# huang-yh/GaussianFormer

Measured on AMD Instinct MI355X. Metric: Gaussians/sec splatted into 200×200×16×18 voxel grid (fwd), higher is better.
Workload: dtype f32

## Files before the change

gaussianformer_amd/csrc/splat_fwd.hip:

```cpp
#include <algorithm>
#include <atomic>
#include <chrono>

#include "gf_common.hpp"

#ifndef GF_TIMELINE
#define GF_TIMELINE 0
#endif
#ifndef GF_X
#define GF_X 0
#endif
#ifndef GF_VD1
#define GF_VD1 1
#endif
#ifndef GF_PHITAB
#define GF_PHITAB 1
#endif
#ifndef GF_STATIC2
#define GF_STATIC2 0
#endif
#ifndef GF_XP
#define GF_XP 0
#endif

// ... 1485 lines not shown
                            for (int k = 0; k < 2; ++k) acc[b0 + k] = __builtin_amdgcn_mfma_f32_32x32x16_f16(sh[kh].v, wh[k][kh].v, acc[b0 + k], 0, 0, 0);
                        }
                    };
                    pair(0);
                    pair(2);
#if GF_TIMELINE
                    asm volatile("" :: "v"(acc[0]), "v"(acc[1]), "v"(acc[2]), "v"(acc[3]));
                    const unsigned long long tg3 = __builtin_amdgcn_s_memtime();
                    tacc[0] += tg1 - tg0; tacc[1] += tg2 - tg1; tacc[2] += tg3 - tg2; tacc[3] += 1;
#endif
                    qhead = (qhead + qn) & (kQCap - 1);
                    qlen -= qn;
                    npend = nnext;
                }
            }
            if (done) {
                if (last_zg && wave == 0) {
                    if (!claim_issued && lane == 0)
                        asm volatile("global_atomic_add %0, %1, %2, off sc0" : "=v"(claimed) : "v"(ctr), "v"(1u) : "memory");
                    asm volatile("s_waitcnt vmcnt(0)" : "+v"(claimed) :: "memory");
                    if (lane == 0) s_next = (int)claimed;
                }
                break;
            }
            __syncthreads();
            __builtin_amdgcn_s_setprio(3);
            list_len = 0;
        }
#if GF_TIMELINE
        if (a.timeline && tid == 0) a.timeline[4 * (size_t)logical + 2] = wall_clock64();
#endif
        if (!LABELS || a.out_logits) {
            typedef __attribute__((address_space(1))) float gfloat;
            typedef float nt4v __attribute__((ext_vector_type(4), aligned(4)));
            typedef __attribute__((address_space(1))) nt4v nt4;
            if ((a.D & 3) == 0) {
                float *stage = &s_stage[wave][0][0];
#pragma unroll
                for (int b = 0; b < 4; ++b) {
                    float *row = stage + ((b >> 1) * 64 + 32 * (b & 1) + n) * kC;
                    *reinterpret_cast<float2 *>(row + 4 * h) = make_float2(acc[b][0], acc[b][1]);
                    *reinterpret_cast<float2 *>(row + 4 * h + 2) = make_float2(acc[b][2], acc[b][3]);
                    *reinterpret_cast<float2 *>(row + 8 + 4 * h) = make_float2(acc[b][4], acc[b][5]);
                    *reinterpret_cast<float2 *>(row + 10 + 4 * h) = make_float2(acc[b][6], acc[b][7]);
                    if (h == 0) *reinterpret_cast<float2 *>(row + 16) = make_float2(acc[b][8], acc[b][9]);
                }
                uint32_t off[10];
                uint32_t okbits = 0u;
#pragma unroll
                for (int it = 0; it < 10; ++it) {
                    const int half = it / 5, i = lane + 64 * (it % 5);
                    const int run = i / kC, k = i - run * kC;
                    const int cx = Xw + (run >> 2), cy = Y0 + (run & 3), Zb = Zw + 4 * half;
                    const bool ok = i < 16 * kC && cx < a.H && cy < a.W && Zb < a.D;
                    okbits |= ok ? (1u << it) : 0u;
                    off[it] = ok ? (uint32_t)((((size_t)cx * a.W + cy) * a.D + Zb) * kC + 4 * k) : 0u;
                }
                asm volatile("" : "+v"(off[0]), "+v"(off[1]), "+v"(off[2]), "+v"(off[3]), "+v"(off[4]), "+v"(off[5]), "+v"(off[6]),
                             "+v"(off[7]), "+v"(off[8]), "+v"(off[9]));
                __builtin_amdgcn_fence(__ATOMIC_ACQ_REL, "wavefront");
                __builtin_amdgcn_wave_barrier();
                gfloat *base = (gfloat *)a.out_logits;
#pragma unroll
                for (int it = 0; it < 10; ++it) {
                    if (okbits & (1u << it)) {
                        const float4 v = *reinterpret_cast<const float4 *>(stage + (it / 5) * 64 * kC + 4 * (lane + 64 * (it % 5)));
                        __builtin_nontemporal_store((nt4v){v.x, v.y, v.z, v.w}, (nt4 *)(base + off[it]));
                    }
                }
            } else {
                float *stage = &s_stage[wave][0][0];
#pragma unroll
                for (int b = 0; b < 4; ++b) {
                    float *row = stage + ((b >> 1) * 64 + 32 * (b & 1) + n) * kC;
#pragma unroll
                    for (int r = 0; r < 10; ++r) {
                        const int c = (r & 3) + 8 * (r >> 2) + 4 * h;
                        if (c < kC) row[c] = acc[b][r];
                    }
                }
                __builtin_amdgcn_fence(__ATOMIC_ACQ_REL, "wavefront");
                __builtin_amdgcn_wave_barrier();
                for (int i = lane; i < 2 * 64 * kC; i += 64) {
                    const int half = i / (64 * kC), l = (i % (64 * kC)) / kC, ch = i % kC;
                    const int cx = Xw + (l >> 4), cy = Y0 + ((l >> 2) & 3), cz = Zw + 4 * half + (l & 3);
                    if (cx < a.H && cy < a.W && cz < a.D) a.out_logits[(((size_t)cx * a.W + cy) * a.D + cz) * kC + ch] = stage[i];
                }
            }
        }
        if (!last_zg) {
            __syncthreads();
        }
#if GF_TIMELINE
        if (a.timeline && tid == 0) a.timeline[4 * (size_t)logical + 3] = wall_clock64();
#endif
    }
#if GF_TIMELINE
    if (a.timeline && lane == 0) {
        unsigned long long *dst = a.timeline + 5 * (size_t)nslots + ((size_t)logical * 4 + wave) * 6;
        dst[0] = tacc[0]; dst[1] = tacc[1]; dst[2] = tacc[2]; dst[3] = tacc[3]; dst[4] = __builtin_amdgcn_s_memtime() - ttile0; dst[5] = tstore;
    }
#endif
    asm volatile("s_waitcnt lgkmcnt(0)\n\ts_barrier" ::: "memory");
    next_local = s_next;
    local = next_local;
    logical = INTER ? local : xcd * per_xcd + local;
    s = INTER ? 8 * (logical / kTilesPerSuper) + xcd : logical / kTilesPerSuper; t = logical % kTilesPerSuper;
    X0 = (s / a.nsy) * kSuper;
    Y0 = (s % a.nsy) * kSuper + t * kTileY;
    if (!(local < per_xcd && (INTER ? s < a.nsx * a.nsy : logical < a.ntiles_total))) break;
    bm = a.bitmask + (size_t)s * a.nrow;
    }
}

struct PhiHotTable { uint32_t w[8][64][4]; };
constexpr uint32_t f16_of_quarters(int k)
{
    if (k == 0) return 0u;
    const uint32_t sign = k < 0 ? 0x8000u : 0u;
    uint32_t m = (uint32_t)(k < 0 ? -k : k);
    int msb = 0;
    for (int i = 0; i < 11; ++i) if (m >> i) msb = i;
    return sign | ((uint32_t)(msb - 2 + 15) << 10) | ((m << (10 - msb)) & 0x3FFu);
}
constexpr PhiHotTable make_phi_hot_table()
{
    PhiHotTable t{};
    for (int lane = 0; lane < 64; ++lane) {
        const int n = lane & 31, h = lane >> 5;
        for (int b = 0; b < 4; ++b) {
            const int lx = 2 * (b & 1) + (n >> 4), ly = (n >> 2) & 3, zz = 4 * (b >> 1) + (n & 3);
            const int x2 = 2 * lx - 3, y2 = 2 * ly - 3, z2 = 2 * zz - 7;
            const int m0[8] = {4, 2 * x2, 2 * y2, 2 * z2, x2 * x2, 0, 0, 0};
            const int m1[8] = {y2 * y2, z2 * z2, x2 * y2, y2 * z2, x2 * z2, 0, 0, 0};
            for (int j = 0; j < 8; ++j) {
                const uint32_t ph = f16_of_quarters(h ? m1[j] : m0[j]);
                const bool one = h ? zz == j : (j < 4 ? lx == j : ly == j - 4);
                const uint32_t ho = one ? 0x3C00u : 0u;
                t.w[b][lane][j >> 1] |= ph << (16 * (j & 1));
                t.w[4 + b][lane][j >> 1] |= ho << (16 * (j & 1));
            }
        }
    }
    return t;
}
__device__ const PhiHotTable kPhiHot = make_phi_hot_table();

constexpr int kWList = 512;
constexpr int kWLdsDwords = 5120;
static_assert(3072 + 2 * kWRow + kQCap + (kC + 1) * kSRow == kWLdsDwords, "LDS map of the wave-autonomous kernel");
static_assert((kWRow + 4 + 3) / 4 <= 3 * 64, "the wave kernel reads its range verdicts with three 16-byte loads per lane");
static_assert(2 * 64 * kC <= 1536 + 3 * kWList, "output staging fits over the slot and the list");

constexpr int kLDense = 576, kLIds = 896;
static_assert(2 * kLDense + kLDense / 2 <= 1536 && 1536 + 3 * kLIds <= 3072 + 2 * kWRow && kLDense % 64 == 0 && kLIds % 64 == 0 && kLIds == kBwdPubLong, "LDS map of the long-row instantiation");
static_assert(kLongWords <= 64 * 64, "one summary bit per word, 64 per lane");
template <bool LABELS, bool PREP = false, bool INTER = true, bool LONG = false>
__global__ __launch_bounds__(64, 2) void gf_splat_render_mfma_wave_kernel(RenderArgs a)
{
    __shared__ __attribute__((aligned(16))) uint32_t s_u[kWLdsDwords];
    float4 *slot = reinterpret_cast<float4 *>(s_u);
    constexpr int kListN = LONG ? kLIds : kWList;
    uint32_t *s_lg = s_u + 1536, *s_blo = s_u + 1536 + kListN, *s_bhi = s_u + 1536 + 2 * kListN;
    float *stage = reinterpret_cast<float *>(s_u);
    unsigned long long *s_row = reinterpret_cast<unsigned long long *>(s_u + 3072);
    uint32_t *s_sum = s_u + 3968;
    uint32_t *q_id = s_u + 3072 + 2 * kWRow;
    float *S = reinterpret_cast<float *>(s_u + 3072 + 2 * kWRow + kQCap);

    const int lane = threadIdx.x;
    const int xcd = (int)(blockIdx.x & 7u);
    const int per_super = 4 * ((a.D + 7) >> 3);
    const int nunits = a.nsx * a.nsy * per_super;
    const int per_xcd = INTER ? ((a.nsx * a.nsy + 7) >> 3) * per_super : (nunits + 7) >> 3;

    const uint32_t m_ps = a.m_ps, m_nsy = a.m_nsy;
    using gptr = const __attribute__((address_space(1))) void *;
    using lptr = __attribute__((address_space(3))) void *;
    int local = (int)(blockIdx.x >> 3);
    bool row_there = false;
    {
        const int logical = INTER ? local : xcd * per_xcd + local;
        const int q0 = (int)__umulhi((uint32_t)logical, m_ps);
        if (local < per_xcd && (INTER ? 8 * q0 + xcd < a.nsx * a.nsy : logical < nunits)) {
            const int s0 = INTER ? 8 * q0 + xcd : q0, r0 = logical - q0 * per_super;
            const int srow0 = a.nsy == 1 ? s0 : (int)__umulhi((uint32_t)s0, m_nsy), scol0 = s0 - srow0 * a.nsy;
            if (srow0 * kSuper + 4 * (r0 & 1) < a.H && scol0 * kSuper + 4 * ((r0 >> 1) & 1) < a.W) {
                if (LONG) {
                    lds_dma16((gptr)(a.summary + (size_t)s0 * a.sum_pitch + 16 * min(lane, (a.sum_pitch >> 4) - 1)), (lptr)s_sum);
                } else {
                    const unsigned long long *bm0 = a.bitmask + (size_t)s0 * a.nrow;
                    for (int i = 0; 128 * i < a.nrow; ++i)
                        if (128 * i + 2 * lane < a.nrow)
                            lds_dma16((gptr)(bm0 + 128 * i + 2 * lane), (lptr)(s_row + 128 * i));
                }
                row_there = true;
            }
        }
    }
    float q0x, q0y, q0z, q1x, q1y, q1z;
    {
        const float *pp = a.pts;
        asm volatile("" : "+v"(pp));
        const size_t ix = a.H > 1 ? 3 * (size_t)a.W * a.D : 0, iy = a.W > 1 ? 3 * (size_t)a.D + 1 : 1, iz = a.D > 1 ? 3 + 2 : 2;
        asm volatile("global_load_dword %0, %6, off\n\tglobal_load_dword %1, %6, off offset:4\n\tglobal_load_dword %2, %6, off offset:8\n\t"
                     "global_load_dword %3, %7, off\n\tglobal_load_dword %4, %8, off\n\tglobal_load_dword %5, %9, off"
                     : "=&v"(q0x), "=&v"(q0y), "=&v"(q0z), "=&v"(q1x), "=&v"(q1y), "=&v"(q1z)
                     : "v"(pp), "v"(pp + ix), "v"(pp + iy), "v"(pp + iz)
                     : "memory");
    }
#if GF_PHITAB
    uint4 phihot_raw[8];
    {
        const uint4 *tp = reinterpret_cast<const uint4 *>(&kPhiHot.w[0][0][0]) + lane;
#pragma unroll
        for (int k = 0; k < 8; ++k) phihot_raw[k] = tp[64 * k];
    }
#endif
    int verdict = 0;
    if (a.verdict_words) {
        const uint4 vw = *reinterpret_cast<const uint4 *>(a.verdict_words);
        const uint32_t vv = (vw.y & 1u) ? vw.w : vw.z;
        verdict = __builtin_amdgcn_readfirstlane((int)(vv & (a.verify_dense ? 15u : 12u)));
        if (blockIdx.x == 0 && lane == 0) {
            a.verdict_words[0] = vw.y;
            a.verdict_words[2 + ((vw.y + 1u) & 1u)] = 0u;
        }
    } else {
        uint32_t v = 0u, rv = 0u;
        uint4 r0 = make_uint4(0, 0, 0, 0), r1 = r0, r2 = r0;
        if (a.range_flags) {
            const uint4 *rp = reinterpret_cast<const uint4 *>(a.range_flags);
            const int last = a.nrange4 - 1;
            r0 = rp[min(lane, last)]; r1 = rp[min(lane + 64, last)]; r2 = rp[min(lane + 128, last)];
        }
        if (a.verify_dense) {
            const uint4 *vp = reinterpret_cast<const uint4 *>(a.verify_flags) + 16 * lane;
#pragma unroll
            for (int k = 0; k < 16; ++k) {
                const uint4 t = vp[k];
                v |= t.x | t.y | t.z | t.w;
            }
        }
        rv = r0.x | r0.y | r0.z | r0.w | r1.x | r1.y | r1.z | r1.w | r2.x | r2.y | r2.z | r2.w;
        rv |= v;
        verdict = (__builtin_amdgcn_ballot_w64((v & 1u) != 0u) ? 1 : 0) | (__builtin_amdgcn_ballot_w64((v & 2u) != 0u) ? 2 : 0) |
                  (__builtin_amdgcn_ballot_w64((rv & 4u) != 0u) ? 4 : 0) | (__builtin_amdgcn_ballot_w64((rv & 8u) != 0u) ? 8 : 0);
    }
    asm volatile("s_waitcnt vmcnt(0)" : "+v"(q0x), "+v"(q0y), "+v"(q0z), "+v"(q1x), "+v"(q1y), "+v"(q1z)::"memory");
    uint32_t rows_ready = 0u;
    if (PREP && blockIdx.x < (unsigned)kRowLayoutBlocks && a.rows_valid && !verdict)
        rows_ready = (LONG ? finish_row_layout_long(a, s_u, lane) : finish_row_layout(a, s_u, lane)) ? 1u : 2u;
    if (blockIdx.x == 0 && lane == 0 && a.state) {
        a.state[0] = (verdict & 1) ? 1u : 0u;
        a.state[1] = verdict ? GF_PATH_ARBITRARY : GF_PATH_MATRIX_CORE_WAVE;
        a.state[2] = (uint32_t)verdict;
        stamp_state(a, rows_ready);
    }
    if (verdict) {
        general_body<GF_SPLAT_BASE, kExpComp, LABELS>(a);
        return;
    }

    const int n = lane & 31, h = lane >> 5;
    for (int i = lane; i < (kC + 1) * kSRow; i += 64) S[i] = 0.f;

    q0x = __builtin_bit_cast(float, __builtin_amdgcn_readfirstlane(__builtin_bit_cast(int, q0x)));
    q0y = __builtin_bit_cast(float, __builtin_amdgcn_readfirstlane(__builtin_bit_cast(int, q0y)));
    q0z = __builtin_bit_cast(float, __builtin_amdgcn_readfirstlane(__builtin_bit_cast(int, q0z)));
    q1x = __builtin_bit_cast(float, __builtin_amdgcn_readfirstlane(__builtin_bit_cast(int, q1x)));
    q1y = __builtin_bit_cast(float, __builtin_amdgcn_readfirstlane(__builtin_bit_cast(int, q1y)));
    q1z = __builtin_bit_cast(float, __builtin_amdgcn_readfirstlane(__builtin_bit_cast(int, q1z)));
    const double p0x = q0x, p0y = q0y, p0z = q0z;
    const double sx = a.H > 1 ? (double)q1x - p0x : 1.0;
    const double sy = a.W > 1 ? (double)q1y - p0y : 1.0;
    const double sz = a.D > 1 ? (double)q1z - p0z : 1.0;

    h8 phi[4], hot[4];
#if GF_PHITAB
#pragma unroll
    for (int b = 0; b < 4; ++b) {
        phi[b] = __builtin_bit_cast(h8, phihot_raw[b]);
        hot[b] = __builtin_bit_cast(h8, phihot_raw[4 + b]);
    }
#else
#pragma unroll
    for (int b = 0; b < 4; ++b) {
        const float ux_ = (float)(2 * (b & 1) + (n >> 4)) - 1.5f, uy_ = (float)((n >> 2) & 3) - 1.5f,
                    uz_ = (float)(4 * (b >> 1) + (n & 3)) - 3.5f;
        const float m0[8] = {1.f, ux_, uy_, uz_, ux_ * ux_, 0.f, 0.f, 0.f};
        const float m1[8] = {uy_ * uy_, uz_ * uz_, ux_ * uy_, uy_ * uz_, ux_ * uz_, 0.f, 0.f, 0.f};
        const int lx = 2 * (b & 1) + (n >> 4), ly = (n >> 2) & 3, zz = 4 * (b >> 1) + (n & 3);
#pragma unroll
        for (int j = 0; j < 8; ++j) {
            phi[b][j] = (_Float16)(h ? m1[j] : m0[j]);
            hot[b][j] = (_Float16)((h ? zz == j : (j < 4 ? lx == j : ly == j - 4)) ? 1.f : 0.f);
        }
    }
#endif

    auto request_records_at = [&](int qh, int start, int count) {
        const uint32_t id = q_id[(qh + start + (n < count ? n : 0)) & (kQCap - 1)];
        const char *rec = reinterpret_cast<const char *>(a.records + (size_t)id * kRecDwords);
        const int o3 = (3 + 3 * h) * 16, o4 = (4 + 3 * h) * 16, o5 = (h ? 7 : 5) * 16;
        char *dst = reinterpret_cast<char *>(slot);
        lds_dma16((gptr)(rec), (lptr)(dst));
        lds_dma16((gptr)(rec + 16), (lptr)(dst + 1024));
        lds_dma16((gptr)(rec + 32), (lptr)(dst + 2048));
        lds_dma16((gptr)(rec + o3), (lptr)(dst + 3072));
        lds_dma16((gptr)(rec + o4), (lptr)(dst + 4096));
        lds_dma16((gptr)(rec + o5), (lptr)(dst + 5120));
    };

    uint32_t *ctr = a.tile_counters + 64 * xcd;
    const int nchunk = (a.nwords + 63) >> 6;
    int nst_prev = 0;
    bool first_unit = true;
    while (true) {
        const int logical = INTER ? local : xcd * per_xcd + local;
        const int qs = (int)__umulhi((uint32_t)logical, m_ps);
        if (!(local < per_xcd && (INTER ? 8 * qs + xcd < a.nsx * a.nsy : logical < nunits))) break;
        bool next_row = false;
        int nst = -1;
        uint32_t claimed = 0u;
        bool have_next = false;
        const int s = INTER ? 8 * qs + xcd : qs, r = logical - qs * per_super;
        const int srow = a.nsy == 1 ? s : (int)__umulhi((uint32_t)s, m_nsy), scol = s - srow * a.nsy;
        const int Xw = srow * kSuper + 4 * (r & 1), Y0 = scol * kSuper + 4 * ((r >> 1) & 1), Zw = 8 * (r >> 2);
        if (Xw < a.H && Y0 < a.W) {
            const unsigned long long *__restrict__ bm = a.bitmask + (size_t)s * a.nrow;
#if GF_TIMELINE
            unsigned long long tl[8] = {(unsigned long long)wall_clock64(), 0, 0, 0, 0, 0, 0, 0};
#endif
            if (!row_there) {
                if (LONG) {
                    lds_dma16((gptr)(a.summary + (size_t)s * a.sum_pitch + 16 * min(lane, (a.sum_pitch >> 4) - 1)), (lptr)s_sum);
                } else {
                    for (int i = 0; 128 * i < a.nrow; ++i)
                        if (128 * i + 2 * lane < a.nrow)
                            lds_dma16((gptr)(bm + 128 * i + 2 * lane), (lptr)(s_row + 128 * i));
                }
            }
            f32x16 acc[4];
#pragma unroll
            for (int b = 0; b < 4; ++b)
#pragma unroll
                for (int q = 0; q < 16; ++q) acc[b][q] = 0.f;
            const double Cx = p0x + ((double)Xw + 1.5) * sx, Cy = p0y + ((double)Y0 + 1.5) * sy, Cz = p0z + ((double)Zw + 3.5) * sz;
            bool published = false;
            int list_len = 0, qlen = 0, qhead = 0, npend = 0;
            if (row_there && nst_prev == 10) asm volatile("s_waitcnt vmcnt(10)" ::: "memory");
            else asm volatile("s_waitcnt vmcnt(0)" ::: "memory");
#if GF_TIMELINE
            tl[1] = wall_clock64();
#endif
            int c = 0, sg = 0;
            int long_lo = 0;
            bool long_first = true;
            if (!LONG) {
                constexpr int kWDense = kWList;
                uint32_t *s_dw = s_u;
                unsigned long long *s_db = reinterpret_cast<unsigned long long *>(s_u + kWDense);
                constexpr int kWPer = (kWRow + 63) / 64;
                const int kw = nchunk;
                unsigned long long wd[kWPer];
                int mine = 0;
#pragma unroll
                for (int k = 0; k < kWPer; ++k) wd[k] = s_row[min(kw * lane + k, kWRow - 1)];
                static_assert(kWPer == 10, "operand list below");
                asm volatile("" : "+v"(wd[0]), "+v"(wd[1]), "+v"(wd[2]), "+v"(wd[3]), "+v"(wd[4]), "+v"(wd[5]), "+v"(wd[6]), "+v"(wd[7]),
                             "+v"(wd[8]), "+v"(wd[9]));
#pragma unroll
                for (int k = 0; k < kWPer; ++k) {
                    const int w = kw * lane + k;
                    wd[k] = (k < kw && w < a.nwords) ? wd[k] : 0ull;
                    mine += wd[k] != 0ull ? 1 : 0;
                }
                const int incl_nz = wave_inclusive_scan(mine);
                const int nd = __builtin_amdgcn_readlane(incl_nz, 63);
                if (nd <= kWDense) {
                    int p = incl_nz - mine;
#pragma unroll
                    for (int k = 0; k < kWPer; ++k) {
                        if (wd[k] != 0ull) {
                            s_dw[p] = (uint32_t)(kw * lane + k);
                            s_db[p] = wd[k];
                            ++p;
                        }
                    }
                }
                if (nd <= kWDense) {
                    __builtin_amdgcn_fence(__ATOMIC_ACQ_REL, "wavefront");
                    __builtin_amdgcn_wave_barrier();
                    int tot = 0;
                    bool fits = true;
                    auto extract = [&](unsigned long long bits, uint32_t id0, int pos) {
                        if (bits) {
                            s_lg[pos++] = id0 + (uint32_t)__builtin_ctzll(bits);
                            bits &= bits - 1;
                        }
                        while (bits) {
                            const int j = __builtin_ctzll(bits);
                            bits &= bits - 1;
                            s_lg[pos++] = id0 + (uint32_t)j;
                        }
                    };
                    if (nd <= 192) {
                        unsigned long long bb[3];
                        uint32_t ii[3];
                        int cn[3], in_[3], tt[3];
#pragma unroll
                        for (int q = 0; q < 3; ++q) {
                            bb[q] = s_db[64 * q + lane];
                            ii[q] = s_dw[64 * q + lane];
                        }
                        asm volatile("" : "+v"(bb[0]), "+v"(bb[1]), "+v"(bb[2]), "+v"(ii[0]), "+v"(ii[1]), "+v"(ii[2]));
#pragma unroll
                        for (int q = 0; q < 3; ++q) {
                            bb[q] = 64 * q + lane < nd ? bb[q] : 0ull;
                            ii[q] *= 64u;
                            cn[q] = __builtin_popcountll(bb[q]);
                        }
#pragma unroll
                        for (int q = 0; q < 3; ++q) in_[q] = wave_inclusive_scan(cn[q]);
#pragma unroll
                        for (int q = 0; q < 3; ++q) tt[q] = __builtin_amdgcn_readlane(in_[q], 63);
                        tot = tt[0] + tt[1] + tt[2];
                        if (tot <= kWList) {
                            extract(bb[0], ii[0], in_[0] - cn[0]);
                            extract(bb[1], ii[1], tt[0] + in_[1] - cn[1]);
                            extract(bb[2], ii[2], tt[0] + tt[1] + in_[2] - cn[2]);
                        } else {
                            fits = false;
                        }
                    } else {
                        for (int d0 = 0; d0 < nd; d0 += 64) {
                            const int i = d0 + lane;
                            const unsigned long long bits = i < nd ? s_db[i] : 0ull;
                            const uint32_t id0 = (i < nd ? s_dw[i] : 0u) * 64u;
                            const int cnt = __builtin_popcountll(bits);
                            const int incl = wave_inclusive_scan(cnt);
                            const int t = __builtin_amdgcn_readlane(incl, 63);
                            if (tot + t > kWList) {
                                fits = false;
                                break;
                            }
                            extract(bits, id0, tot + incl - cnt);
                            tot += t;
                        }
                    }
                    if (fits) {
                        list_len = tot;
                        c = nchunk;
                    }
                }
            }
            while (true) {
                bool last = false;
                if (LONG) {
                    uint32_t *d_lo = s_u, *d_hi = s_u + kLDense;
                    unsigned short *d_w = reinterpret_cast<unsigned short *>(s_u + 2 * kLDense);
                    if (!long_first) {
                        lds_dma16((gptr)(a.summary + (size_t)s * a.sum_pitch + 16 * min(lane, (a.sum_pitch >> 4) - 1)), (lptr)s_sum);
                        asm volatile("s_waitcnt vmcnt(0)" ::: "memory");
                    }
                    long_first = false;
                    const uint4 sv = reinterpret_cast<const uint4 *>(s_sum)[lane];
                    auto nib16 = [](uint32_t d) -> uint32_t {
                        uint32_t x = d & 0x0F0F0F0Fu;
                        x = (x | (x >> 4)) & 0x00FF00FFu;
                        return (x | (x >> 8)) & 0x0000FFFFu;
                    };
                    unsigned long long sm = (unsigned long long)(nib16(sv.x) | (nib16(sv.y) << 16)) |
                                            ((unsigned long long)(nib16(sv.z) | (nib16(sv.w) << 16)) << 32);
                    {
                        const int left = a.nwords - 64 * lane;
                        sm = left >= 64 ? sm : (left > 0 ? sm & bits_below(left) : 0ull);
                    }
                    const int cw = __builtin_popcountll(sm);
                    const int incl_w = wave_inclusive_scan(cw);
                    const int nd = __builtin_amdgcn_readlane(incl_w, 63);
                    const int cnt = min(nd - long_lo, kLDense);
                    {
                        unsigned long long m = sm;
                        int t = incl_w - cw - long_lo;
                        while (m) {
                            const int b = __builtin_ctzll(m);
                            m &= m - 1;
                            if ((unsigned)t < (unsigned)cnt) d_w[t] = (unsigned short)(64 * lane + b);
                            ++t;
                        }
                    }
                    __builtin_amdgcn_fence(__ATOMIC_ACQ_REL, "wavefront");
                    __builtin_amdgcn_wave_barrier();
                    const uint32_t *bm32 = reinterpret_cast<const uint32_t *>(bm);
                    for (int k0 = 0; k0 < cnt; k0 += 64) {
                        const uint32_t w = d_w[min(k0 + lane, cnt - 1)];
                        lds_dma4((gptr)(bm32 + 2 * w), (lptr)(d_lo + k0));
                        lds_dma4((gptr)(bm32 + 2 * w + 1), (lptr)(d_hi + k0));
                    }
                    asm volatile("s_waitcnt vmcnt(0)" ::: "memory");
                    int tot = 0, used = 0;
                    for (int k0 = 0; k0 < cnt; k0 += 64) {
                        const int j = k0 + lane;
                        const bool in = j < cnt;
                        const int jc = min(j, cnt - 1);
                        unsigned long long bits = (unsigned long long)d_lo[jc] | ((unsigned long long)d_hi[jc] << 32);
                        bits = in ? bits : 0ull;
                        const uint32_t id0 = (uint32_t)d_w[jc] * 64u;
                        const int cb = __builtin_popcountll(bits);
                        const int incl = wave_inclusive_scan(cb);
                        const int total = __builtin_amdgcn_readlane(incl, 63);
                        int pos = -1, adm = 64;
                        if (tot + total <= kLIds) {
                            pos = tot + incl - cb;
                        } else {
                            adm = 0;
                            int e_adm = 0;
                            for (int g8 = 0; g8 < 8; ++g8) {
                                const int e1 = __builtin_amdgcn_readlane(incl, 8 * g8 + 7);
                                if (tot + e1 > kLIds) break;
                                adm = 8 * (g8 + 1);
                                e_adm = e1;
                            }
                            if (lane < adm) pos = tot + incl - cb;
                            (void)e_adm;
                        }
                        if (pos >= 0) {
                            while (bits) {
                                const int b = __builtin_ctzll(bits);
                                bits &= bits - 1;
                                s_lg[pos++] = id0 + (uint32_t)b;
                            }
                        }
                        if (adm == 64) {
                            tot += total;
                            used += min(64, cnt - k0);
                        } else {
                            tot += adm ? __builtin_amdgcn_readlane(incl, max(adm - 1, 0)) : 0;
                            used += min(adm, cnt - k0);
                            break;
                        }
                    }
                    list_len = tot;
                    last = long_lo + used >= nd;
                    long_lo += used;
                }
                while (!LONG) {
                    if (c >= nchunk) {
                        last = true;
                        break;
                    }
                    const int w = 64 * c + lane;
                    unsigned long long bits = w < a.nwords ? s_row[w] : 0ull;
                    const int cnt = __builtin_popcountll(bits);
                    const int incl = wave_inclusive_scan(cnt);
                    const int total = __builtin_amdgcn_readlane(incl, 63);
                    int pos = -1;
                    if (total <= kWList) {
                        if (list_len + total > kWList) break;
                        pos = list_len + incl - cnt;
                        list_len += total;
                        ++c;
                    } else {
                        bool full = false;
                        for (; sg < 8; ++sg) {
                            const int e1 = __builtin_amdgcn_readlane(incl, 8 * sg + 7);
                            const int e0 = sg ? __builtin_amdgcn_readlane(incl, 8 * sg - 1) : 0;
                            if (list_len + (e1 - e0) > kWList) {
                                full = true;
                                break;
                            }
                            if ((lane >> 3) == sg) pos = list_len + (incl - cnt) - e0;
                            list_len += e1 - e0;
                        }
                        if (!full) {
                            sg = 0;
                            ++c;
                        }
                        if (pos >= 0) {
                            const uint32_t id0 = (uint32_t)w * 64u;
                            while (bits) {
                                const int j = __builtin_ctzll(bits);
                                bits &= bits - 1;
                                s_lg[pos++] = id0 + (uint32_t)j;
                            }
                        }
                        if (full) break;
                        continue;
                    }
                    const uint32_t id0 = (uint32_t)w * 64u;
                    while (bits) {
                        const int j = __builtin_ctzll(bits);
                        bits &= bits - 1;
                        s_lg[pos++] = id0 + (uint32_t)j;
                    }
                }
                __builtin_amdgcn_fence(__ATOMIC_ACQ_REL, "wavefront");
                __builtin_amdgcn_wave_barrier();
#if GF_TIMELINE
                if (!tl[2]) tl[2] = wall_clock64();
#endif
                for (int b0 = 0; b0 < list_len; b0 += 64) {
                    const uint32_t id = s_lg[min(b0 + lane, list_len - 1)];
                    lds_dma4((gptr)(&a.boxes[id].x), (lptr)(s_blo + b0));
                    lds_dma4((gptr)(&a.boxes[id].y), (lptr)(s_bhi + b0));
                }
                asm volatile("s_waitcnt vmcnt(0)" ::: "memory");
                if (PREP && a.rows_valid && r == 0 && !published) {
                    published = true;
                    constexpr int kPub = LONG ? kBwdPubLong : kBwdList;
                    if (last && list_len <= kPub) {
                        uint32_t *dst = a.pub_lists + (size_t)s * (3 * kPub);
                        for (int i = lane; i < list_len; i += 64) {
                            dst[i] = s_lg[i]; dst[kPub + i] = s_blo[i]; dst[2 * kPub + i] = s_bhi[i];
                        }
                        if (lane == 0) a.pub_len[s] = (uint32_t)list_len;
                    } else if (lane == 0) {
                        if (LONG) a.pub_len[s] = 0xFFFFFFFFu;
                        else atomicOr(const_cast<uint32_t *>(a.verify_flags) + (kListsBad - 64), 1u);
                    }
                }
#if GF_TIMELINE
                if (!tl[3]) tl[3] = wall_clock64();
#endif
                const int nbase = list_len + ((LONG && !last) ? 64 : 0);
                for (int base = 0; base < nbase || (last && base == 0); base += 64) {
                    const int i = base + lane;
                    const int ic = min(i, max(list_len - 1, 0));
                    const uint32_t eg = s_lg[ic];
                    const uint32_t blo = s_blo[ic], bhi = s_bhi[ic];
                    const bool hit = i < list_len && ux(blo) < Xw + 4 && ux(bhi) > Xw && uy(blo) < Y0 + 4 && uy(bhi) > Y0 &&
                                     uz(blo) < Zw + 8 && uz(bhi) > Zw;
                    const unsigned long long todo = __builtin_amdgcn_ballot_w64(hit);
                    if (hit) q_id[(qhead + qlen + (int)mbcnt(todo)) & (kQCap - 1)] = eg;
                    qlen += __builtin_popcountll(todo);
                    const bool final_batch = last && base + 64 >= list_len;
                    const bool flush = LONG && !last && base >= list_len;
                    while (true) {
                        if (npend == 0) {
                            if (!(qlen >= 32 || (final_batch && qlen > 0))) break;
                            npend = min(qlen, 32);
                            __builtin_amdgcn_fence(__ATOMIC_ACQ_REL, "wavefront");
                            __builtin_amdgcn_wave_barrier();
                            request_records_at(qhead, 0, npend);
                        }
                        const int avail = qlen - npend;
                        if (!(avail >= 32 || final_batch || flush)) break;
                        const int qn = npend;
                        asm volatile("s_waitcnt vmcnt(0)" ::: "memory");
#if GF_TIMELINE
                        if (!tl[4]) tl[4] = wall_clock64();
                        tl[7] += 1;
#endif
                        const bool live = n < qn;
                        const float4 r0 = slot[lane], r1 = slot[64 + lane], r2 = slot[128 + lane];
                        const float4 e0 = slot[192 + lane], e1 = slot[256 + lane], e2 = slot[320 + lane];
                        __builtin_amdgcn_fence(__ATOMIC_ACQ_REL, "wavefront");
                        __builtin_amdgcn_wave_barrier();
                        const int nnext = (flush && avail < 32) ? 0 : min(avail, 32);
                        if (nnext > 0) request_records_at(qhead, qn, nnext);
                        const bool last_group = final_batch && nnext == 0;
                        if (last_group && lane == 0 && !(GF_STATIC2 && first_unit))
                            asm volatile("global_atomic_add %0, %1, %2, off sc0" : "=v"(claimed) : "v"(ctr), "v"(1u) : "memory");
                            {
                            const float opa = live ? r0.w : 0.f;
                            const float v[12] = {e0.x, e0.y, e0.z, e0.w, e1.x, e1.y, e1.z, e1.w, e2.x, e2.y, e2.z, e2.w};
                            if (h == 0) {
#pragma unroll
                                for (int k = 0; k < 12; ++k) S[k * kSRow + n] = opa * v[k];
                            } else {
#pragma unroll
                                for (int k = 0; k < 6; ++k) S[(12 + k) * kSRow + n] = opa * v[k];
                            }
                        }
                        H8 t1, t2, t3;
                        {
                            const double L = 1.4426950408889634074;
                            const double c0 = r1.x, c1 = r1.y, c2 = r1.z, c3 = r1.w, c4 = r2.x, c5 = r2.y;
                            double th[5];
                            if (h == 0) {
                                const double ex = Cx - (double)r0.x, ey = Cy - (double)r0.y, ez = Cz - (double)r0.z;
                                const double gx = c0 * ex + c3 * ey + c5 * ez, gy = c3 * ex + c1 * ey + c4 * ez, gz = c5 * ex + c4 * ey + c2 * ez;
                                th[0] = -0.5 * L * (ex * gx + ey * gy + ez * gz);
                                th[1] = -L * sx * gx; th[2] = -L * sy * gy; th[3] = -L * sz * gz;
                                th[4] = -0.5 * L * sx * sx * c0;
                            } else {
                                th[0] = -0.5 * L * sy * sy * c1; th[1] = -0.5 * L * sz * sz * c2;
                                th[2] = -L * sx * sy * c3; th[3] = -L * sy * sz * c4; th[4] = -L * sx * sz * c5;
                            }
#pragma unroll
                            for (int j = 0; j < 5; ++j) split3(live ? th[j] : 0.0, t1.e[j], t2.e[j], t3.e[j]);
#pragma unroll
                            for (int j = 5; j < 8; ++j) { t1.e[j] = (_Float16)0.f; t2.e[j] = (_Float16)0.f; t3.e[j] = (_Float16)0.f; }
                        }
                        H8 tb;
                        {
                            const uint32_t glo = __float_as_uint(r2.z), ghi = __float_as_uint(r2.w);
                            const int x0 = ux(glo) - Xw, x1 = ux(ghi) - Xw, y0 = uy(glo) - Y0, y1 = uy(ghi) - Y0;
                            const int z0 = uz(glo) - Zw, z1 = uz(ghi) - Zw;
#pragma unroll
                            for (int j = 0; j < 8; ++j) {
                                const bool in = h ? (j >= z0 && j < z1) : (j < 4 ? (j >= x0 && j < x1) : (j - 4 >= y0 && j - 4 < y1));
                                tb.e[j] = (_Float16)((in && live) ? 0.f : -32768.f);
                            }
                        }
                        __builtin_amdgcn_fence(__ATOMIC_ACQ_REL, "wavefront");
                        __builtin_amdgcn_wave_barrier();
                        H8 sh[2], sl[2];
#pragma unroll
                        for (int q = 0; q < 4; ++q) {
                            const float4 v4 = *reinterpret_cast<const float4 *>(S + min(n, kC) * kSRow + 8 * q + 4 * h);
                            const fp16x2 ha = __builtin_amdgcn_cvt_pkrtz(v4.x, v4.y), hb = __builtin_amdgcn_cvt_pkrtz(v4.z, v4.w);
                            const fp16x2 la = __builtin_amdgcn_cvt_pkrtz(__builtin_fmaf((float)ha[0], -1.0f, v4.x), __builtin_fmaf((float)ha[1], -1.0f, v4.y));
                            const fp16x2 lb = __builtin_amdgcn_cvt_pkrtz(__builtin_fmaf((float)hb[0], -1.0f, v4.z), __builtin_fmaf((float)hb[1], -1.0f, v4.w));
                            sh[q >> 1].p[2 * (q & 1)] = ha; sh[q >> 1].p[2 * (q & 1) + 1] = hb;
                            sl[q >> 1].p[2 * (q & 1)] = la; sl[q >> 1].p[2 * (q & 1) + 1] = lb;
                        }
                        auto pair = [&](int b0) {
                            f32x16 d0, d1;
#pragma unroll
                            for (int q = 0; q < 16; ++q) { d0[q] = 0.f; d1[q] = 0.f; }
                            d0 = __builtin_amdgcn_mfma_f32_32x32x16_f16(t3.v, phi[b0], d0, 0, 0, 0);
                            d1 = __builtin_amdgcn_mfma_f32_32x32x16_f16(t3.v, phi[b0 + 1], d1, 0, 0, 0);
                            d0 = __builtin_amdgcn_mfma_f32_32x32x16_f16(t2.v, phi[b0], d0, 0, 0, 0);
                            d1 = __builtin_amdgcn_mfma_f32_32x32x16_f16(t2.v, phi[b0 + 1], d1, 0, 0, 0);
                            d0 = __builtin_amdgcn_mfma_f32_32x32x16_f16(t1.v, phi[b0], d0, 0, 0, 0);
                            d1 = __builtin_amdgcn_mfma_f32_32x32x16_f16(t1.v, phi[b0 + 1], d1, 0, 0, 0);
                            d0 = __builtin_amdgcn_mfma_f32_32x32x16_f16(tb.v, hot[b0], d0, 0, 0, 0);
                            d1 = __builtin_amdgcn_mfma_f32_32x32x16_f16(tb.v, hot[b0 + 1], d1, 0, 0, 0);
                            H8 wh[2][2], wl[2][2];
                            auto weights = [&](const f32x16 &d, int k) {
#pragma unroll
                                for (int q = 0; q < 16; q += 2) {
                                    const float w0 = __builtin_amdgcn_exp2f(d[q]), w1 = __builtin_amdgcn_exp2f(d[q + 1]);
                                    const fp16x2 hi = __builtin_amdgcn_cvt_pkrtz(w0, w1);
                                    float q0, q1;
                                    asm("v_fma_mix_f32 %0, %1, -1.0, %2 op_sel_hi:[1,0,0]" : "=v"(q0) : "v"(hi), "v"(w0));
                                    asm("v_fma_mix_f32 %0, %1, -1.0, %2 op_sel:[1,0,0] op_sel_hi:[1,0,0]" : "=v"(q1) : "v"(hi), "v"(w1));
                                    wh[k][q >> 3].p[(q & 7) >> 1] = hi;
                                    wl[k][q >> 3].p[(q & 7) >> 1] = __builtin_amdgcn_cvt_pkrtz(q0, q1);
                                }
                            };
                            weights(d0, 0);
                            weights(d1, 1);
#pragma unroll
                            for (int kh = 0; kh < 2; ++kh) {
#pragma unroll
                                for (int k = 0; k < 2; ++k) acc[b0 + k] = __builtin_amdgcn_mfma_f32_32x32x16_f16(sl[kh].v, wh[k][kh].v, acc[b0 + k], 0, 0, 0);
#pragma unroll
                                for (int k = 0; k < 2; ++k) acc[b0 + k] = __builtin_amdgcn_mfma_f32_32x32x16_f16(sh[kh].v, wl[k][kh].v, acc[b0 + k], 0, 0, 0);
#pragma unroll
                                for (int k = 0; k < 2; ++k) acc[b0 + k] = __builtin_amdgcn_mfma_f32_32x32x16_f16(sh[kh].v, wh[k][kh].v, acc[b0 + k], 0, 0, 0);
                            }
                        };
                        pair(0);
                        pair(2);
                        have_next = have_next || last_group;
                        qhead = (qhead + qn) & (kQCap - 1);
                        qlen -= qn;
                        npend = nnext;
                    }
                }
                if (last) break;
                list_len = 0;
            }
#if GF_TIMELINE
            asm volatile("" :: "v"(acc[0]), "v"(acc[1]), "v"(acc[2]), "v"(acc[3]));
            tl[5] = wall_clock64();
#endif
            if (!have_next && lane == 0 && !(GF_STATIC2 && first_unit))
                asm volatile("global_atomic_add %0, %1, %2, off sc0" : "=v"(claimed) : "v"(ctr), "v"(1u) : "memory");
            asm volatile("s_waitcnt vmcnt(0)" : "+v"(claimed)::"memory");
            if (GF_STATIC2 && first_unit) claimed = (uint32_t)local + (gridDim.x >> 3);
            have_next = true;
            {
                const int nl = __builtin_amdgcn_readfirstlane((int)claimed), nlog = INTER ? nl : xcd * per_xcd + nl;
                const int q2 = (int)__umulhi((uint32_t)nlog, m_ps);
                if (nl < per_xcd && (INTER ? 8 * q2 + xcd < a.nsx * a.nsy : nlog < nunits)) {
                    const int s2 = INTER ? 8 * q2 + xcd : q2, r2 = nlog - q2 * per_super;
                    const int srow2 = a.nsy == 1 ? s2 : (int)__umulhi((uint32_t)s2, m_nsy), scol2 = s2 - srow2 * a.nsy;
                    if (srow2 * kSuper + 4 * (r2 & 1) < a.H && scol2 * kSuper + 4 * ((r2 >> 1) & 1) < a.W) {
                        if (LONG) {
                            lds_dma16((gptr)(a.summary + (size_t)s2 * a.sum_pitch + 16 * min(lane, (a.sum_pitch >> 4) - 1)), (lptr)s_sum);
                        } else {
                            const unsigned long long *bm2 = a.bitmask + (size_t)s2 * a.nrow;
                            for (int i = 0; 128 * i < a.nrow; ++i)
                                if (128 * i + 2 * lane < a.nrow)
                                    lds_dma16((gptr)(bm2 + 128 * i + 2 * lane), (lptr)(s_row + 128 * i));
                        }
                        next_row = true;
                    }
                }
            }
            typedef __attribute__((address_space(1))) float gfloat;
            typedef float nt4v __attribute__((ext_vector_type(4), aligned(4)));
            typedef __attribute__((address_space(1))) nt4v nt4;
            if ((a.D & 3) == 0) {
#pragma unroll
                for (int b = 0; b < 4; ++b) {
                    float *row = stage + ((b >> 1) * 64 + 32 * (b & 1) + n) * kC;
                    *reinterpret_cast<float2 *>(row + 4 * h) = make_float2(acc[b][0], acc[b][1]);
                    *reinterpret_cast<float2 *>(row + 4 * h + 2) = make_float2(acc[b][2], acc[b][3]);
                    *reinterpret_cast<float2 *>(row + 8 + 4 * h) = make_float2(acc[b][4], acc[b][5]);
                    *reinterpret_cast<float2 *>(row + 10 + 4 * h) = make_float2(acc[b][6], acc[b][7]);
                    if (h == 0) *reinterpret_cast<float2 *>(row + 16) = make_float2(acc[b][8], acc[b][9]);
                }
                auto labels_from_stage = [&]() {
#pragma unroll
                    for (int half = 0; half < 2; ++half) {
                        const int l = lane;
                        const float *row = stage + (64 * half + l) * kC;
                        float best = row[0];
                        int arg = 0;
#pragma unroll
                        for (int ch = 1; ch < kC; ++ch) {
                            const float v = row[ch];
                            if (v > best) { best = v; arg = ch; }
                        }
                        const int cx = Xw + (l >> 4), cy = Y0 + ((l >> 2) & 3), cz = Zw + 4 * half + (l & 3);
                        if (cx < a.H && cy < a.W && cz < a.D) a.out_labels[((size_t)cx * a.W + cy) * a.D + cz] = arg;
                    }
                };
                if (LABELS) {
                    __builtin_amdgcn_fence(__ATOMIC_ACQ_REL, "wavefront");
                    __builtin_amdgcn_wave_barrier();
                    labels_from_stage();
                }
                if (!LABELS || a.out_logits) {
                uint32_t off[10];
                uint32_t okbits = 0u;
#pragma unroll
                for (int j = 0; j < 5; ++j) {
                    const int i = lane + 64 * j;
                    const int run = i / kC, k = i - run * kC;
                    const int cx = Xw + (run >> 2), cy = Y0 + (run & 3);
                    const bool okc = i < 16 * kC && cx < a.H && cy < a.W;
                    const uint32_t o = (uint32_t)((((size_t)cx * a.W + cy) * a.D + Zw) * kC + 4 * k);
#pragma unroll
                    for (int half = 0; half < 2; ++half) {
                        const bool ok = okc && Zw + 4 * half < a.D;
                        okbits |= ok ? (1u << (5 * half + j)) : 0u;
                        off[5 * half + j] = ok ? o + 4 * kC * half : 0u;
                    }
                }
                nst = ((!LABELS) && Xw + 4 <= a.H && Y0 + 4 <= a.W && Zw + 8 <= a.D) ? 10 : -1;
                asm volatile("" : "+v"(off[0]), "+v"(off[1]), "+v"(off[2]), "+v"(off[3]), "+v"(off[4]), "+v"(off[5]), "+v"(off[6]),
                             "+v"(off[7]), "+v"(off[8]), "+v"(off[9]));
                __builtin_amdgcn_fence(__ATOMIC_ACQ_REL, "wavefront");
                __builtin_amdgcn_wave_barrier();
                gfloat *obase = (gfloat *)a.out_logits;
                float4 val[10];
#pragma unroll
                for (int it = 0; it < 10; ++it)
                    val[it] = *reinterpret_cast<const float4 *>(stage + (it / 5) * 64 * kC + 4 * (lane + 64 * (it % 5)));
#pragma unroll
                for (int it = 0; it < 10; ++it) {
                    if (okbits & (1u << it))
                        __builtin_nontemporal_store((nt4v){val[it].x, val[it].y, val[it].z, val[it].w}, (nt4 *)(obase + off[it]));
                }
                }
            } else {
#pragma unroll
                for (int b = 0; b < 4; ++b) {
                    float *row = stage + ((b >> 1) * 64 + 32 * (b & 1) + n) * kC;
#pragma unroll
                    for (int q = 0; q < 10; ++q) {
                        const int ch = (q & 3) + 8 * (q >> 2) + 4 * h;
                        if (ch < kC) row[ch] = acc[b][q];
                    }
                }
                __builtin_amdgcn_fence(__ATOMIC_ACQ_REL, "wavefront");
                __builtin_amdgcn_wave_barrier();
                if (!LABELS || a.out_logits)
                    for (int i = lane; i < 2 * 64 * kC; i += 64) {
                        const int half = i / (64 * kC), l = (i % (64 * kC)) / kC, ch = i % kC;
                        const int cx = Xw + (l >> 4), cy = Y0 + ((l >> 2) & 3), cz = Zw + 4 * half + (l & 3);
                        if (cx < a.H && cy < a.W && cz < a.D) a.out_logits[(((size_t)cx * a.W + cy) * a.D + cz) * kC + ch] = stage[i];
                    }
                if (LABELS) {
#pragma unroll
                    for (int half = 0; half < 2; ++half) {
                        const int l = lane;
                        const float *row = stage + (64 * half + l) * kC;
                        float best = row[0];
                        int arg = 0;
                        for (int ch = 1; ch < kC; ++ch) {
                            const float v = row[ch];
                            if (v > best) { best = v; arg = ch; }
                        }
                        const int cx = Xw + (l >> 4), cy = Y0 + ((l >> 2) & 3), cz = Zw + 4 * half + (l & 3);
                        if (cx < a.H && cy < a.W && cz < a.D) a.out_labels[((size_t)cx * a.W + cy) * a.D + cz] = arg;
                    }
                }
            }
            asm volatile("s_waitcnt lgkmcnt(0)" ::: "memory");
#if GF_TIMELINE
            tl[6] = wall_clock64();
            if (a.timeline && lane == 0)
#pragma unroll
                for (int k = 0; k < 8; ++k) a.timeline[8 * (size_t)logical + k] = tl[k];
#endif
        }
        if (!have_next) {
            if (lane == 0 && !(GF_STATIC2 && first_unit)) asm volatile("global_atomic_add %0, %1, %2, off sc0" : "=v"(claimed) : "v"(ctr), "v"(1u) : "memory");
            asm volatile("s_waitcnt vmcnt(0)" : "+v"(claimed)::"memory");
            if (GF_STATIC2 && first_unit) claimed = (uint32_t)local + (gridDim.x >> 3);
        }
        local = __builtin_amdgcn_readfirstlane((int)claimed);
        row_there = next_row;
        nst_prev = nst;
        first_unit = false;
    }
}

static int mfma_wave_grid(int nunits)
{
    static int cus = 0;
    if (cus == 0) {
        int dev = 0, n = 0;
        if (hipGetDevice(&dev) != hipSuccess || hipDeviceGetAttribute(&n, hipDeviceAttributeMultiprocessorCount, dev) != hipSuccess || n <= 0) n = 256;
        cus = n;
    }
    const int per_xcd = (nunits + 7) / 8;
    return 8 * std::min(per_xcd, std::max(1, 8 * cus / 8));
}

#if GF_DEV
#include "splat_fwd_pair.inc"
#include "splat_fwd_solo.inc"
#endif

struct BoxVolArgs {
    const int *means_int;
    const int *radii;
    uint32_t *tiles_touched;
    unsigned long long *num_rendered;
    int P, H, W, D, per_axis;
};

__global__ __launch_bounds__(256) void gf_box_volumes_kernel(BoxVolArgs a)
{
    const int g = blockIdx.x * 256 + threadIdx.x;
    uint32_t vol = 0;
    if (g < a.P) {
        int lo[3], hi[3];
        gaussian_box(a.means_int, a.radii, a.per_axis, g, a.H, a.W, a.D, lo, hi);
        vol = (uint32_t)(hi[2] - lo[2]) * (uint32_t)(hi[1] - lo[1]) * (uint32_t)(hi[0] - lo[0]);
        a.tiles_touched[g] = vol;
    }
    unsigned long long s = vol;
#pragma unroll
    for (int d = 32; d >= 1; d >>= 1) s += __shfl_xor(s, d, 64);
    if (lane_id() == 0 && s) atomicAdd(a.num_rendered, s);
}

static int mfma_grid(int ntiles_total)
{
    static int cus = 0;
    if (cus == 0) {
        int dev = 0, n = 0;
        if (hipGetDevice(&dev) != hipSuccess || hipDeviceGetAttribute(&n, hipDeviceAttributeMultiprocessorCount, dev) != hipSuccess || n <= 0) n = 256;
        cus = n;
    }
    const int per_xcd = (ntiles_total + 7) / 8;
    return 8 * std::min(per_xcd, std::max(1, 2 * cus / 8));
}

static int mfma_wave_units(int nsuper, int D) { return nsuper * 4 * ((D + 7) / 8); }

static bool mfma_by_wave(int nrow)
{
    return nrow <= kWRow && option(kOptSplatTileKernel) == 0;
}
static bool mfma_by_wave_long(int nrow, int nwords, int flags)
{
    return GF_VD1 && nrow > kWRow && nwords <= kLongWords && (flags & GF_WORKSPACE_ZEROED) && option(kOptSplatTileKernel) == 0;
}

static int mfma_kind(int nrow, int D, int P, bool labels, bool prepare_backward, int flags = 0)
{
#if GF_DEV
    const bool plain = !labels && !prepare_backward && nrow <= kPRowMax && (D & 3) == 0 && option(kOptSplatTileKernel) == 0;
    if (plain && dev_option(kOptSplatPair) && P < (1 << 20)) return 2;
    if (plain && dev_option(kOptSplatSolo) && P < (1 << 16)) return 3;
#else
    (void)D; (void)P; (void)labels; (void)prepare_backward;
#endif
    return (mfma_by_wave(nrow) || mfma_by_wave_long(nrow, (P + 63) / 64, flags)) ? 1 : 0;
}
#if GF_DEV
static int solo_waves() { return dev_option(kOptSplatSoloWaves) == 3 ? 3 : 2; }
#endif

static uint32_t mfma_counter_init(int kind, int nsuper, int nrow, int D)
{
#if GF_DEV
    if (kind == 3)
        return (uint32_t)((solo_waves() == 3 ? mfma_solo_grid<3>(mfma_wave_units(nsuper, D), nrow) : mfma_solo_grid<2>(mfma_wave_units(nsuper, D), nrow)) / 8);
    if (kind == 2) return (uint32_t)(mfma_pair_grid(mfma_wave_units(nsuper, D), nrow) / 8);
#else
    (void)nrow;
#endif
    return kind == 1 ? (uint32_t)((GF_STATIC2 ? 2 : 1) * (mfma_wave_grid(mfma_wave_units(nsuper, D)) / 8)) : (uint32_t)(mfma_grid(nsuper * kTilesPerSuper) / 8);
}

static void launch_render_mfma(const RenderArgs &r, int nsuper, hipStream_t stream)
{
    hipEvent_t ev0, ev1;
    const bool prof = profile_slot(&ev0, &ev1);
    if (prof) (void)hipEventRecord(ev0, stream);
    const int kind = mfma_kind(r.nrow, r.D, r.P, r.out_labels != nullptr, r.rows_valid != 0u, r.summary ? GF_WORKSPACE_ZEROED : 0);
    const int wave_grid = mfma_wave_grid(mfma_wave_units(nsuper, r.D));
#if GF_DEV
    if (kind == 3 && solo_waves() == 3)
        hipLaunchKernelGGL((gf_splat_render_mfma_solo_kernel<3, false>), dim3(mfma_solo_grid<3>(mfma_wave_units(nsuper, r.D), r.nrow)), dim3(64), solo_lds_bytes(r.nrow), stream, r, FusedArgs{});
    else if (kind == 3)
        hipLaunchKernelGGL((gf_splat_render_mfma_solo_kernel<2, false>), dim3(mfma_solo_grid<2>(mfma_wave_units(nsuper, r.D), r.nrow)), dim3(64), solo_lds_bytes(r.nrow), stream, r, FusedArgs{});
    else if (kind == 2)
        hipLaunchKernelGGL(gf_splat_render_mfma_pair_kernel, dim3(mfma_pair_grid(mfma_wave_units(nsuper, r.D), r.nrow)), dim3(128), pair_lds_bytes(r.nrow), stream, r);
// ... 337 lines not shown
```

Baseline: 640.0 million.

## Rebalance record slices across half-waves and vectorize box-mask construction

Changes which 16-byte record chunks each half-wave fetches, so both halves now write 10 semantic values into the shared S buffer with a uniform stride instead of 12 and 6. The per-lane box mask is built with packed 16-bit integer compare and shift tricks rather than eight scalar compares and selects. The high/low fp16 split residual uses v_fma_mix instructions that read the half inputs directly, avoiding explicit converts. This depends on the record layout matching the new offsets, which is not visible here.

Result: faster. 681.7 million (median of 6 runs) (+6.5%).

```diff
diff --git a/gaussianformer_amd/csrc/splat_fwd.hip b/gaussianformer_amd/csrc/splat_fwd.hip
--- a/gaussianformer_amd/csrc/splat_fwd.hip
+++ b/gaussianformer_amd/csrc/splat_fwd.hip
@@ -1811,7 +1811,7 @@
     auto request_records_at = [&](int qh, int start, int count) {
         const uint32_t id = q_id[(qh + start + (n < count ? n : 0)) & (kQCap - 1)];
         const char *rec = reinterpret_cast<const char *>(a.records + (size_t)id * kRecDwords);
-        const int o3 = (3 + 3 * h) * 16, o4 = (4 + 3 * h) * 16, o5 = (h ? 7 : 5) * 16;
+        const int o3 = (3 + 2 * h) * 16, o4 = (4 + 2 * h) * 16, o5 = (5 + 2 * h) * 16;
         char *dst = reinterpret_cast<char *>(slot);
         lds_dma16((gptr)(rec), (lptr)(dst));
         lds_dma16((gptr)(rec + 16), (lptr)(dst + 1024));
@@ -2172,16 +2172,11 @@
                         const bool last_group = final_batch && nnext == 0;
                         if (last_group && lane == 0 && !(GF_STATIC2 && first_unit))
                             asm volatile("global_atomic_add %0, %1, %2, off sc0" : "=v"(claimed) : "v"(ctr), "v"(1u) : "memory");
-                            {
+                        {
                             const float opa = live ? r0.w : 0.f;
-                            const float v[12] = {e0.x, e0.y, e0.z, e0.w, e1.x, e1.y, e1.z, e1.w, e2.x, e2.y, e2.z, e2.w};
-                            if (h == 0) {
-#pragma unroll
-                                for (int k = 0; k < 12; ++k) S[k * kSRow + n] = opa * v[k];
-                            } else {
-#pragma unroll
-                                for (int k = 0; k < 6; ++k) S[(12 + k) * kSRow + n] = opa * v[k];
-                            }
+                            const float v[10] = {e0.x, e0.y, e0.z, e0.w, e1.x, e1.y, e1.z, e1.w, e2.x, e2.y};
+#pragma unroll
+                            for (int k = 0; k < 10; ++k) S[(8 * h + k) * kSRow + n] = opa * v[k];
                         }
                         H8 t1, t2, t3;
                         {
@@ -2208,10 +2203,18 @@
                             const uint32_t glo = __float_as_uint(r2.z), ghi = __float_as_uint(r2.w);
                             const int x0 = ux(glo) - Xw, x1 = ux(ghi) - Xw, y0 = uy(glo) - Y0, y1 = uy(ghi) - Y0;
                             const int z0 = uz(glo) - Zw, z1 = uz(ghi) - Zw;
-#pragma unroll
-                            for (int j = 0; j < 8; ++j) {
-                                const bool in = h ? (j >= z0 && j < z1) : (j < 4 ? (j >= x0 && j < x1) : (j - 4 >= y0 && j - 4 < y1));
-                                tb.e[j] = (_Float16)((in && live) ? 0.f : -32768.f);
+                            typedef short i16x2 __attribute__((ext_vector_type(2)));
+                            auto dup = [](int v) { return i16x2{(short)v, (short)v}; };
+                            const i16x2 lo_a = dup(h ? z0 : x0), hi_a = dup((h ? z1 : x1) - 1);
+                            const i16x2 lo_b = dup(h ? z0 : y0), hi_b = dup((h ? z1 : y1) - 1);
+                            const short j4 = h ? 4 : 0;
+                            const i16x2 dead = dup(live ? 0 : -1);
+#pragma unroll
+                            for (int k = 0; k < 4; ++k) {
+                                const short j0 = (short)(2 * (k & 1)) + (k < 2 ? (short)0 : j4);
+                                const i16x2 jj = i16x2{j0, (short)(j0 + 1)};
+                                const i16x2 out = ((jj - (k < 2 ? lo_a : lo_b)) | ((k < 2 ? hi_a : hi_b) - jj) | dead) >> (short)15;
+                                tb.u[k] = __builtin_bit_cast(uint32_t, out) & 0xF800F800u;
                             }
                         }
                         __builtin_amdgcn_fence(__ATOMIC_ACQ_REL, "wavefront");
@@ -2221,10 +2224,13 @@
                         for (int q = 0; q < 4; ++q) {
                             const float4 v4 = *reinterpret_cast<const float4 *>(S + min(n, kC) * kSRow + 8 * q + 4 * h);
                             const fp16x2 ha = __builtin_amdgcn_cvt_pkrtz(v4.x, v4.y), hb = __builtin_amdgcn_cvt_pkrtz(v4.z, v4.w);
-                            const fp16x2 la = __builtin_amdgcn_cvt_pkrtz(__builtin_fmaf((float)ha[0], -1.0f, v4.x), __builtin_fmaf((float)ha[1], -1.0f, v4.y));
-                            const fp16x2 lb = __builtin_amdgcn_cvt_pkrtz(__builtin_fmaf((float)hb[0], -1.0f, v4.z), __builtin_fmaf((float)hb[1], -1.0f, v4.w));
+                            float ra0, ra1, rb0, rb1;
+                            asm("v_fma_mix_f32 %0, %1, -1.0, %2 op_sel_hi:[1,0,0]" : "=v"(ra0) : "v"(ha), "v"(v4.x));
+                            asm("v_fma_mix_f32 %0, %1, -1.0, %2 op_sel:[1,0,0] op_sel_hi:[1,0,0]" : "=v"(ra1) : "v"(ha), "v"(v4.y));
+                            asm("v_fma_mix_f32 %0, %1, -1.0, %2 op_sel_hi:[1,0,0]" : "=v"(rb0) : "v"(hb), "v"(v4.z));
+                            asm("v_fma_mix_f32 %0, %1, -1.0, %2 op_sel:[1,0,0] op_sel_hi:[1,0,0]" : "=v"(rb1) : "v"(hb), "v"(v4.w));
                             sh[q >> 1].p[2 * (q & 1)] = ha; sh[q >> 1].p[2 * (q & 1) + 1] = hb;
-                            sl[q >> 1].p[2 * (q & 1)] = la; sl[q >> 1].p[2 * (q & 1) + 1] = lb;
+                            sl[q >> 1].p[2 * (q & 1)] = __builtin_amdgcn_cvt_pkrtz(ra0, ra1); sl[q >> 1].p[2 * (q & 1) + 1] = __builtin_amdgcn_cvt_pkrtz(rb0, rb1);
                         }
                         auto pair = [&](int b0) {
                             f32x16 d0, d1;
```
